# Rajwardhan0511/LLM-Based-Apache-Spark-Optimization

Hardware: AMD Instinct MI355X
Metric: output_tokens_per_sec (higher is better)
Workload: dtype bf16; 1 GPU; model=duckdb-nsql-7B, global_batch=32, seq_len=256, prompt_len=128, parallelism=dp1, decode=greedy

## Files before the change

csrc/bindings.cpp:

```cpp
#ifdef LSA_BINDINGS_SELFTEST
#include <ATen/ATen.h>
#include <hip/hip_runtime_api.h>
#else
#include <torch/extension.h>
#include <c10/hip/HIPStream.h>
#include <hip/hip_runtime.h>
#endif

#include "kernels/gemm_sk.h"
#include "kernels/lsa_epi.h"

extern "C" {
int lsa_gemm(const void* X, int ldx, int M, int K, const void* Wf, int N, void* out, int epi, int nb, int splitk,
             hipStream_t stream);
int lsa_add_rmsnorm(float* h, const float* parts, int nparts, long part_stride, const int* ids, const void* emb,
                    const int* row_idx, int write_h, const void* w, float eps, void* xn, int rows, int D,
                    int xf_mt, long long* ss_out, int ss_ld, int ss_nzero, void* x8, float* sx8, hipStream_t s);
int lsa_prefetch(const void* const* ptrs, const long* bytes, int nr, int wgs, hipStream_t s);
int lsa_res_add_ss(float* h, const float* parts, int nparts, long part_stride, void* xn, int rows, int D, int xf_mt,
                   long long* ss_out, hipStream_t s);
int lsa_a8_gemm(const void* X8, const void* s8, const float* sx, int M, int K, const void* Wq, const float* wscale,
                const void* Sw, int wk, int N, void* out, void* out_s8, int epi, int nb, int splitk, int waves, int depth,
                int xfo, const LsaEpi* ep, hipStream_t stream);
int lsa_quant_xf8(const void* x, int ldx, int M, int K, int MT, void* x8, float* sx, hipStream_t s);
// ... 85 lines not shown
int lsa_ar_alloc(size_t bytes, void** out);
int lsa_ar_free(void* p);
int lsa_ar_handle(void* p, char* out64);
int lsa_ar_open(const char* in64, void** out);
int lsa_ar_close(void* p);
int lsa_ar_max_world();
int lsa_prefill_qblock();
int lsa_ar_wallclock_khz(int* out);
int lsa_ar_header_bytes();
int lsa_ar_run(float* data, long n, float* out, uint8_t* const* regions, int rank, int world, size_t maxb,
               int nblocks, long long timeout_ticks, int* err, int nslab, long slab_stride, const float* res_h,
               void* res_xn, long long* res_ss, int res_d, int res_xmt, int mode, hipStream_t s);
int lsa_fp4_gemm_ex(const void* X, int ldx, int M, int K, const void* Wq, const void* S, int N, void* out, int epi,
                    int nb, int splitk, int waves, int xfrag, const LsaEpi* ep, hipStream_t stream);
int lsa_fp4_dequant(const void* Wq, const void* S, int N, int K, void* Wf, hipStream_t s);
}

namespace {

#ifdef LSA_BINDINGS_SELFTEST
hipStream_t cur_stream() { return nullptr; }
bool on_dev(const at::Tensor& t) { return t.defined(); }
#else
hipStream_t cur_stream() { return c10::hip::getCurrentHIPStream().stream(); }
bool on_dev(const at::Tensor& t) { return t.is_cuda(); }
#endif

void check(int rc, const char* what) { TORCH_CHECK(rc == 0, "lsa kernel '", what, "' failed: rc=", rc); }

void need(const at::Tensor& t, at::ScalarType dt, const char* name) {
// ... 141 lines not shown
             const c10::optional<at::Tensor>& rowss, double eps, const c10::optional<at::Tensor>& h,
             const c10::optional<at::Tensor>& xout, int64_t xmt, const c10::optional<at::Tensor>& ss_out, const c10::optional<at::Tensor>& tickets) {
  need(xf, at::kBFloat16, "xf");
  need(wf, at::kBFloat16, "wf");
  TORCH_CHECK(M >= 1 && M <= 64 && K % 32 == 0, "gemm_xf: M in 1..64, K % 32 == 0");
  const int64_t mt = M <= 16 ? 1 : (M <= 32 ? 2 : 4);
  TORCH_CHECK(xf.is_contiguous() && xf.numel() >= mt * 16 * K, "xf too small for M=", M, " K=", K);
  TORCH_CHECK(wf.numel() == N * K, "weight numel mismatch");
  check_out(epi, out, splitk, M, N, mt);
  const EpiOpts eo = epi_opts(epi, M, N, K, rowss, eps, h, xout, xmt, ss_out, tickets, N / 16);
  check(lsa_gemm_ex(xf.data_ptr(), K, M, K, wf.data_ptr(), N, out.data_ptr(), epi, nb, splitk, waves, div, 2,
                    eo.on ? &eo.e : nullptr, cur_stream()),
        "gemm_xf");
}


void fp8_gemm_xf(const at::Tensor& xf, int64_t M, int64_t K, const at::Tensor& wq, const at::Tensor& wscale, int64_t N,
                 at::Tensor& out, int64_t epi, int64_t nb, int64_t splitk, int64_t waves, int64_t depth,
                 const c10::optional<at::Tensor>& rowss,
                 double eps, const c10::optional<at::Tensor>& h, const c10::optional<at::Tensor>& xout, int64_t xmt,
                 const c10::optional<at::Tensor>& ss_out, const c10::optional<at::Tensor>& tickets) {
  need(xf, at::kBFloat16, "xf");
  need(wscale, at::kFloat, "wscale");
  TORCH_CHECK(on_dev(wq) && wq.element_size() == 1 && wq.numel() == N * K, "wq must be N*K fp8 bytes");
  TORCH_CHECK(M >= 1 && M <= 64 && K % 64 == 0, "fp8_gemm_xf: M in 1..64, K % 64 == 0");
  const int64_t mt = M <= 16 ? 1 : (M <= 32 ? 2 : 4);
  TORCH_CHECK(xf.is_contiguous() && xf.numel() >= mt * 16 * K, "xf too small");
  check_out(epi, out, splitk, M, N, mt);
  const EpiOpts eo = epi_opts(epi, M, N, K, rowss, eps, h, xout, xmt, ss_out, tickets, N / 16);
  lsa_fp8_gemm_knobs((int)waves, (int)depth);
// ... 926 lines not shown
                   (int)res_xmt, (int)mode, cur_stream()),
        "ar_run");
}

}

#ifndef LSA_BINDINGS_SELFTEST
PYBIND11_MODULE(TORCH_EXTENSION_NAME, m) {
  m.doc() = "gfx950 HIP kernels for the MI355X NL->SQL / Spark-error inference engine";
  m.def("gemm", &gemm, py::arg("x"), py::arg("wf"), py::arg("N"), py::arg("out"), py::arg("epi"), py::arg("nb"),
        py::arg("splitk"), py::arg("waves") = 4, py::arg("div") = 4, py::arg("xlds") = 0,
        py::arg("rowss") = py::none(), py::arg("eps") = 1e-5, py::arg("h") = py::none(), py::arg("xout") = py::none(), py::arg("xmt") = 0, py::arg("ss_out") = py::none(), py::arg("tickets") = py::none());
  m.def("gemm_xf", &gemm_xf, py::arg("xf"), py::arg("M"), py::arg("K"), py::arg("wf"), py::arg("N"), py::arg("out"),
        py::arg("epi"), py::arg("nb"), py::arg("splitk"), py::arg("waves") = 4, py::arg("div") = 4,
        py::arg("rowss") = py::none(), py::arg("eps") = 1e-5, py::arg("h") = py::none(), py::arg("xout") = py::none(), py::arg("xmt") = 0, py::arg("ss_out") = py::none(), py::arg("tickets") = py::none());
  m.def("gemm_sk", &gemm_sk, py::arg("x"), py::arg("wf"), py::arg("N"), py::arg("out"), py::arg("epi"), py::arg("ws"),
        py::arg("tickets"), py::arg("ncu"), py::arg("min_share") = 0, py::arg("cfg") = -1, py::arg("xf") = 0,
        py::arg("rows") = 0);
  m.def("gemm_sk_rope", &gemm_sk_rope, py::arg("x"), py::arg("wf"), py::arg("ws"), py::arg("tickets"), py::arg("ncu"),
        py::arg("min_share"), py::arg("cfg"), py::arg("pos"), py::arg("tok_seq"), py::arg("block_tables"),
        py::arg("cos_t"), py::arg("sin_t"), py::arg("q_out"), py::arg("kc"), py::arg("vc"), py::arg("H"), py::arg("Hkv"),
        py::arg("xf") = 0, py::arg("rows") = 0);
  m.def("gemm_sk_epilogue", [](int64_t mode) { lsa_gemm_sk_epilogue((int)mode); });
  m.def("gemm_sk_nbuf", [](int64_t n) { lsa_gemm_sk_nbuf((int)n); });
  m.def("gemm_sk_one_phase", [](int64_t on) { lsa_gemm_sk_one_phase((int)on); });
  m.def("rmsnorm_xf_tile_min", [](int64_t rows) { lsa_rmsnorm_xf_tile_min((int)rows); });
  m.def("gemm_sk_ws_bytes", [](int64_t ncu) { return lsa_gemm_sk_ws_bytes((int)ncu); });
  m.def("gemm_sk_tickets", [](int64_t ncu) { return (int64_t)lsa_gemm_sk_tickets((int)ncu); });
  m.def("fp4_gemm", &fp4_gemm, py::arg("x"), py::arg("wq"), py::arg("sw"), py::arg("N"), py::arg("out"), py::arg("epi"),
        py::arg("nb"), py::arg("splitk"), py::arg("waves") = 4, py::arg("rowss") = py::none(), py::arg("eps") = 1e-5,
// ... 105 lines not shown
```

llm_based_apache_spark_optimization_amd/engine/runner.py:

```python
from __future__ import annotations


import math
import os
from typing import Optional, Sequence

import torch

from .. import ops
from ..models.llama import LlamaWeights
from ..ops import reference as ref

BLOCK = 64
REPEAT_WINDOW = 64
RR_DECODE = os.environ.get("LSA_RR", "1") != "0"


class TPCommError(RuntimeError):
    """A TP peer missed a one-shot all-reduce (the kernel poisoned the result with NaN and set err)."""


class ModelRunner:
    def __init__(self, weights: LlamaWeights, max_slots: int = 32, max_model_len: int = 4096,
                 num_kv_blocks: Optional[int] = None, kv_memory_fraction: float = 0.85,
                 max_new_cap: Optional[int] = None, tp=None, use_graphs: bool = True,
                 fuse_rope: Optional[bool] = None, seq_parallel: Optional[bool] = None, sp_min_tokens: Optional[int] = None,
                 kv_dtype: Optional[str] = None, spec_tokens: int = 0, spec_ngram: tuple = (3, 1),
                 spec_quantized: bool = False, spec_guided: bool = False, spec_sampled: bool = False):
        self.w = weights
        self.spec_tokens = int(spec_tokens)
# ... 102 lines not shown
        a8d = self.a8 and self.a8_down_ok
        self.x8d = torch.zeros(xr * self.ffn_l if a8d else 1, dtype=torch.uint8, device=dev)
        self.s8d = torch.full((mt64 * 64 * (self.ffn_l // 128) if a8d else 1,), 127, dtype=torch.uint8, device=dev)
        self.o_buf = torch.zeros(8 * S * self.d, **f32)
        self.down_buf = torch.zeros(8 * S * self.d, **f32)
        self.qkv_buf = torch.zeros(8 * S * (self.H + 2 * self.Hkv) * self.D, **f32)
        self.logits_l = torch.zeros(S, self.Vl, **f32)
        self.logits = self.logits_l if tps == 1 else torch.zeros(S, self.V, **f32)
        self.gather_buf = None if tps == 1 else torch.zeros(tps * S * self.Vl, **f32)
        nsplit_max = max(4, ops.decode_split_plan(1, self.Hkv, self.max_model_len)[1])
        self.attn_ws = ops.decode_workspace(S, self.H, self.Hkv, nsplit_max, dev)
        self.amax_part = torch.zeros(S * ((self.V + 4095) // 4096), dtype=torch.int64, device=dev)
        self.cand = torch.zeros(S * ((self.V + 2047) // 2048) * 64, dtype=torch.int64, device=dev)
        self.fused_norm = tps == 1 and all(lw.norms_folded for lw in weights.layers)
        self.fused_norm_max_batch = 16 if self.d >= 4096 else 0
        self.res_cfg = None
        self.ssq = torch.zeros(2 * self.L + 2, S, dtype=torch.int64, device=dev)
        self.res_tickets = torch.zeros(max(64, self.d // 16), dtype=torch.int32, device=dev)
        self.wide_norm = all(lw.norms_folded for lw in weights.layers)
        self._plan_rr()
        self.zero_slab = torch.zeros(1, 1, self.d, **f32)
        self.h_alt = torch.zeros(1, self.d, **f32)
        self.graphs: dict = {}
        self._pending_bt: dict = {}
        self.park_past_prompt = False
        self.guided = False
        self._g_host_on: set = set()
        if self.tp is not None and self.tp.size > 1 and self.on_gpu:
            self.tp.warmup()
            if not self.tp.capturable():
# ... 46 lines not shown
    def _a8_splitk_b1(self) -> int:
        kind = self.w.layers[0].wqkv.kind
        if kind not in ("fp8", "mxfp4"):
            return 1
        ak = "fp8a" if kind == "fp8" else "fp4a"
        return max(ops.pick_gemm_config(1, self.d, K, "f32", xf=True, kind=ak)[1] for K in (self.H * self.D, self.ffn_l))

    def oracle_plan(self, B: int) -> dict:
        plan = dict(zip(("qkv", "gate_up", "o", "down"), self.a8_plan(B)))
        plan["rr"] = B == 1 and self.rr_decode and self.rr_a8
        return plan

    def use_xfrag(self, B: int) -> bool:
        return self.on_gpu and 16 < B <= 64 and self.w.layers[0].wqkv.kind in ("bf16", "fp8", "mxfp4")

    def _lm_head(self, xn: torch.Tensor, M: int, xf: bool = False) -> torch.Tensor:
        loc = self.logits_l[:M] if M <= self.max_slots else torch.empty(M, self.Vl, dtype=torch.float32,
                                                                         device=self.device)
        if xf:
            ops.linear_xf(xn, M, self.w.lm_head, "f32", out=loc, splitk=1)
        else:
            ops.linear(xn, self.w.lm_head, "f32", out=loc, splitk=1)
        return self._gather_logits(loc, M)

    def _gather_logits(self, loc: torch.Tensor, M: int) -> torch.Tensor:
        if self.tp is None or self.tp.size == 1:
            return loc
        tps = self.tp.size
        gb = self.gather_buf[: tps * M * self.Vl] if M <= self.max_slots else torch.empty(
            tps * M * self.Vl, dtype=torch.float32, device=self.device)
        self.tp.all_gather(gb, loc.reshape(-1))
        full = self.logits[:M] if M <= self.max_slots else torch.empty(M, self.V, dtype=torch.float32,
                                                                      device=self.device)
        full.view(M, tps, self.Vl).copy_(gb.view(tps, M, self.Vl).transpose(0, 1))
        return full
# ... 29 lines not shown
        wna = self.wide_norm and not a8
        wnm = self.wide_norm and not a8m
        raw0 = wna or wnm
        ssq = self.ssq
        rn_a = lambda l: dict(rownorm=(ssq[2 * l], self.eps)) if (wna or (l == 0 and raw0)) else {}
        assert not (a8 and wna), "a W8A8 qkv input comes from the quantising norm launch"
        rn_m = lambda l: dict(rownorm=(ssq[2 * l + 1], self.eps)) if wnm else {}
        o_parts = self.o_buf[: sk_o * B * d].view(sk_o, B, d)
        d_parts = self.down_buf[: sk_d * B * d].view(sk_d, B, d)
        qkv_parts = self.qkv_buf[: sk_q * B * nqkv].view(sk_q, B, nqkv)
        plan = plan or ops.decode_split_plan(B, self.Hkv, self.max_model_len)
        ws = self.attn_ws
        if xf:
            xn, attn, act = self.xn_f, self.attn_f, self.act_f

            def lin(x, wt, epi, **kw):
                return ops.linear_xf(x, B, wt, epi, **kw)
        else:
            xn, attn, act = self.xn[:B], self.attn[:B], self.act[:B]
            lin = ops.linear
        for l, lw in enumerate(w.layers):
            if l == 0 and raw0:
                ops.add_rmsnorm(h, lw.attn_norm, self.eps, xn, ids=ids, emb=w.embed, rows=B, xf=xf,
                                ss_out=ssq.view(-1), ss_ld=self.max_slots, ss_nzero=2 * self.L, **q8)
            elif l == 0:
                ops.add_rmsnorm(h, lw.attn_norm, self.eps, xn, ids=ids, emb=w.embed, rows=B, xf=xf, **q8)
            elif wna:
                self._reduce_add(d_parts, h, xn, ssq[2 * l], B, xf)
            else:
                ops.add_rmsnorm(h, lw.attn_norm, self.eps, xn, parts=self._reduce_parts(d_parts), rows=B, xf=xf, **q8)
            if a8:
                ops.linear_a8(self.x8, self.sx8, B, lw.wqkv, "f32", out=qkv_parts, splitk=sk_q, **rn_a(l))
            else:
                lin(xn, lw.wqkv, "f32", out=qkv_parts, splitk=sk_q, **rn_a(l))
            kc, vc = self.kv[l, 0], self.kv[l, 1]
# ... 12 lines not shown
                lin(attn, lw.wo, "f32", out=o_parts, splitk=sk_o)
            if wnm:
                self._reduce_add(o_parts, h, xn, ssq[2 * l + 1], B, xf)
            else:
                ops.add_rmsnorm(h, lw.mlp_norm, self.eps, xn, parts=self._reduce_parts(o_parts), rows=B, xf=xf, **q8m)
            if a8m:
                ops.linear_a8(self.x8, self.sx8, B, lw.w_gate_up, "silu", out=self.x8d if a8d else act,
                              out_s8=self.s8d if a8d else None)
            else:
                lin(xn, lw.w_gate_up, "silu", out=act, **rn_m(l))
            if a8d:
                ops.linear_a8(self.x8d, None, B, lw.w_down, "f32", out=d_parts, splitk=sk_d, s8=self.s8d)
            else:
                lin(act, lw.w_down, "f32", out=d_parts, splitk=sk_d)
        ops.add_rmsnorm(h, w.final_norm, self.eps, xn, parts=self._reduce_parts(d_parts), rows=B, xf=xf)
        self._decode_tail(B, sample, xn, xf, guided)

    def _decode_step_fused(self, B: int, sample: bool, plan: Optional[tuple] = None, guided: bool = False) -> None:
        w, d = self.w, self.d
        ids, pos, bt = self.input_ids[:B], self.positions[:B], self.block_tables[:B]
        h = self.h[:B]
        xf = self.use_xfrag(B)
        nqkv = (self.H + 2 * self.Hkv) * self.D
        sk_q = self._splitk(B, d, nqkv, tp_reduced=False, xf=xf)
        sk_o = ops.pick_gemm_config(B, d, self.H * self.D, "res", xf=xf, kind=w.layers[0].wo.kind)[1]
        sk_d = ops.pick_gemm_config(B, d, self.ffn_l, "res", xf=xf, kind=w.layers[0].w_down.kind)[1]
        rc = {}
        if self.res_cfg is not None:
            nb_, sk_o, wv_, dv_ = self.res_cfg
            sk_d = sk_o
            rc = dict(nb=nb_, waves=wv_, div=dv_)
# ... 73 lines not shown
                ops.linear_a8_rr(hs[cur], o_parts, hs[1 - cur], lw.w_gate_up, "silu", out=self.x8d, out_s8=self.s8d,
                                 eps=self.eps)
                cur = 1 - cur
                ops.linear_a8(self.x8d, None, 1, lw.w_down, "f32", out=d_parts, splitk=sk_d, s8=self.s8d)
                continue
            ops.attn_decode(self.q[:1], kc, vc, bt, pos, self.H, self.Hkv, self.scale, attn.view(1, self.H, self.D),
                            workspace=self.attn_ws, plan=plan, qkv_parts=qkv_parts, cos=self.cos, sin=self.sin,
                            kv_scales=self._kv_scales(l), rownorm=rn)
            ops.linear(attn, lw.wo, "f32", out=o_parts, splitk=sk_o)
            ops.linear_rr(hs[cur], o_parts, hs[1 - cur], lw.w_gate_up, "silu", out=act, eps=self.eps)
            cur = 1 - cur
            ops.linear(act, lw.w_down, "f32", out=d_parts, splitk=sk_d)
        ops.add_rmsnorm(hs[cur], w.final_norm, self.eps, xn, parts=d_parts, rows=1, write_h=False)
        self._decode_tail(B, sample, xn, False, guided)

    def _decode_tail(self, B: int, sample: bool, xn, xf: bool, guided: bool = False) -> None:
        logits = self._lm_head(xn, B, xf)
        if guided:
            self._dfa_mask(logits, self.gen_len[:B], self.input_ids[:B], self.finished[:B])
        st = (self.out_tokens[:B], self.gen_len[:B], self.input_ids[:B], self.positions[:B], self.finished[:B])
        if sample:
            ops.sample_commit(logits, self.hist[:B], self.penalty[:B], self.temperature[:B], self.top_k[:B],
                              self.top_p[:B], self.seeds[:B], *st, self.eos, self.limit[:B], self.eos_on[:B],
                              workspace=(self.amax_part, self.cand) if self.on_gpu else None,
                              last_n=self.last_n[:B])
        else:
            ops.argmax_commit(logits, *st, self.eos, self.limit[:B], self.eos_on[:B],
                              part=self.amax_part if self.on_gpu else None)

    def final_hidden(self, B: int) -> torch.Tensor:
        if self.step_xfrag(B):
            return ops.from_xfrag(self.xn_f, B, self.d)
# ... 678 lines not shown
```

llm_based_apache_spark_optimization_amd/models/llama.py:

```python
from __future__ import annotations

import dataclasses
import math
import glob
import json
import os
from typing import Optional

import torch

from .. import ops
from .spec import ModelSpec, spec_from_hf_config


FOLD_NORMS = True


@dataclasses.dataclass
class LayerWeights:
    wqkv: ops.PackedWeight
    wo: ops.PackedWeight
    w_gate_up: ops.PackedWeight
    w_down: ops.PackedWeight
    attn_norm: torch.Tensor
# ... 42 lines not shown
def pack_layer(spec: ModelSpec, wq, wk, wv, wo, wg, wu, wd, an, mn, rank=0, tp=1, kind="bf16") -> LayerWeights:
    hd = spec.head_dim
    hq, hk = spec.n_heads // tp, spec.n_kv_heads // tp
    q = wq.view(spec.n_heads, hd, -1)[rank * hq:(rank + 1) * hq].reshape(hq * hd, -1)
    k = wk.view(spec.n_kv_heads, hd, -1)[rank * hk:(rank + 1) * hk].reshape(hk * hd, -1)
    v = wv.view(spec.n_kv_heads, hd, -1)[rank * hk:(rank + 1) * hk].reshape(hk * hd, -1)
    wqkv = torch.cat([q, k, v], 0)
    wo_s = _shard_cols(wo, rank, tp)
    gu = ops.interleave_gate_up(_shard_rows(wg, rank, tp), _shard_rows(wu, rank, tp))
    wd_s = _shard_cols(wd, rank, tp)
    an, mn = an.to(torch.bfloat16), mn.to(torch.bfloat16)
    if FOLD_NORMS:
        wqkv = (wqkv.float() * an.float()[None, :]).to(torch.bfloat16)
        gu = (gu.float() * mn.float()[None, :]).to(torch.bfloat16)
        an, mn = torch.ones_like(an), torch.ones_like(mn)
    P = ops.PackedWeight.from_dense
    return LayerWeights(P(wqkv.contiguous(), kind), P(wo_s.contiguous(), kind), P(gu.contiguous(), kind),
                        P(wd_s.contiguous(), kind), an.contiguous(),
                        mn.contiguous(), norms_folded=FOLD_NORMS)


def init_random(spec: ModelSpec, device="cpu", seed: int = 0, kind: str = "bf16", std: float = 0.02,
                tp_rank: int = 0, tp_size: int = 1) -> LlamaWeights:
    check_tp(spec, tp_size)
    dev = torch.device(device)
    g = torch.Generator(device=dev).manual_seed(seed)
    d, hd = spec.hidden, spec.head_dim

    def rnd(*shape, s=std):
        return (torch.randn(*shape, generator=g, device=dev, dtype=torch.float32) * s).to(torch.bfloat16)

# ... 3 lines not shown
    embed = rnd(spec.vocab_size, d, s=1.0)
    layers = []
    for _ in range(spec.n_layers):
        wq = rnd(spec.n_heads * hd, d)
        wk = rnd(spec.n_kv_heads * hd, d)
        wv = rnd(spec.n_kv_heads * hd, d)
        wo = rnd(d, spec.n_heads * hd)
        wg = rnd(spec.ffn, d)
        wu = rnd(spec.ffn, d)
        wd = rnd(d, spec.ffn)
        layers.append(pack_layer(spec, wq, wk, wv, wo, wg, wu, wd, ones(d), ones(d), tp_rank, tp_size, kind))
        del wq, wk, wv, wo, wg, wu, wd
    final_norm = ones(d)
    head = embed if spec.tie_embeddings else rnd(spec.vocab_size, d)
    lm_head = ops.PackedWeight.from_dense(_shard_rows(head, tp_rank, tp_size).contiguous(), kind)
    return LlamaWeights(spec, embed, layers, final_norm, lm_head, tp_rank, tp_size)


def from_hf_state_dict(spec: ModelSpec, sd: dict, device="cpu", kind: str = "bf16", tp_rank: int = 0,
                       tp_size: int = 1) -> LlamaWeights:
    check_tp(spec, tp_size)
    dev = torch.device(device)

    def t(name):
        return sd[name].to(device=dev, dtype=torch.bfloat16)

    layers = []
    for i in range(spec.n_layers):
        p = f"model.layers.{i}."
        layers.append(pack_layer(
            spec, t(p + "self_attn.q_proj.weight"), t(p + "self_attn.k_proj.weight"), t(p + "self_attn.v_proj.weight"),
            t(p + "self_attn.o_proj.weight"), t(p + "mlp.gate_proj.weight"), t(p + "mlp.up_proj.weight"),
            t(p + "mlp.down_proj.weight"), t(p + "input_layernorm.weight"), t(p + "post_attention_layernorm.weight"),
            tp_rank, tp_size, kind))
    embed = t("model.embed_tokens.weight").contiguous()
    head = embed if (spec.tie_embeddings or "lm_head.weight" not in sd) else t("lm_head.weight")
    lm_head = ops.PackedWeight.from_dense(_shard_rows(head, tp_rank, tp_size).contiguous(), kind)
    return LlamaWeights(spec, embed, layers, t("model.norm.weight").contiguous(), lm_head, tp_rank, tp_size)


def load_safetensors_dir(path: str, device="cpu", kind="bf16", name: Optional[str] = None,
                         template: Optional[str] = None, tp_rank=0, tp_size=1) -> LlamaWeights:
    from safetensors.torch import load_file

    from .spec import get_spec

    with open(os.path.join(path, "config.json")) as f:
        cfg = json.load(f)
    if template is None:
        try:
            template = get_spec(name).template if name else "raw"
        except KeyError:
# ... 103 lines not shown
```

llm_based_apache_spark_optimization_amd/ops/__init__.py:

```python
from __future__ import annotations

import dataclasses
import importlib
import importlib.util
import json
import math
import os
from typing import NamedTuple, Optional

import torch

from . import reference as ref

_ext = None
_ext_err: Optional[BaseException] = None

EPI = {"bf16": 0, "f32": 1, "silu": 2, "res": 3}


def ext():
    global _ext, _ext_err
    if _ext is None and _ext_err is None:
        try:
            alt = os.environ.get("LSA_HIP_SO")
# ... 124 lines not shown
    sp[:, :kb] = sl
    return wq, sp.view(N // 16, kb4, 4, 64).permute(0, 1, 3, 2).contiguous()


def dequantize_mxfp4(wq: torch.Tensor, sw: torch.Tensor, N: int, K: int) -> torch.Tensor:
    kb = K // 128
    packed = wq.reshape(N // 16, kb, 4, 16, 16).permute(0, 3, 1, 2, 4).reshape(N, K // 2)
    codes = torch.stack([packed & 15, packed >> 4], dim=-1).view(N, K).long()
    vals = torch.tensor(FP4_VALUES, device=wq.device)[codes & 7] * (1.0 - 2.0 * (codes >> 3).float())
    sb = sw.reshape(N // 16, -1, 64, 4).permute(0, 1, 3, 2).reshape(N // 16, -1, 64)[:, :kb]
    sb = sb.reshape(N // 16, kb, 4, 16).permute(0, 3, 1, 2).reshape(N, K // 32).float()
    scale = torch.where(sb > 0, torch.exp2(sb - 127.0), torch.zeros_like(sb))
    return (vals.view(N, K // 32, 32) * scale[..., None]).view(N, K)


@dataclasses.dataclass
class PackedWeight:

    N: int
    K: int
    kind: str
    data: torch.Tensor
    scale: Optional[torch.Tensor] = None
    requested: Optional[str] = None

    @staticmethod
    def from_dense(w: torch.Tensor, kind: str = "bf16") -> "PackedWeight":
        N, K = w.shape
        if not w.is_cuda:
            return PackedWeight(N, K, "dense", w.to(torch.bfloat16).contiguous(), None, kind)
        if kind == "fp8":
            q, s = quantize_fp8(w)
            return PackedWeight(N, K, "fp8", q, s.contiguous())
        if kind == "mxfp4":
            wq, sw = pack_mxfp4(*quantize_mxfp4(w))
            return PackedWeight(N, K, "mxfp4", wq, sw)
        wb = w.to(torch.bfloat16)
        return PackedWeight(N, K, "bf16", shuffle_weight(wb))

# ... 403 lines not shown
def to_xfrag(x: torch.Tensor) -> torch.Tensor:
    M, K = x.shape
    mt = xfrag_tiles(M)
    xp = torch.zeros(mt * 16, K, dtype=x.dtype, device=x.device)
    xp[:M] = x
    return xp.view(mt, 16, K // 32, 4, 8).permute(2, 0, 3, 1, 4).contiguous().view(-1)


def from_xfrag(xf: torch.Tensor, M: int, K: int) -> torch.Tensor:
    mt = xfrag_tiles(M)
    return xf[: mt * 16 * K].view(K // 32, mt, 4, 16, 8).permute(1, 3, 0, 2, 4).reshape(mt * 16, K)[:M]


def linear_xf(xf: torch.Tensor, M: int, w: PackedWeight, epi: str = "bf16", out: Optional[torch.Tensor] = None,
              splitk: Optional[int] = None, nb: Optional[int] = None, waves: Optional[int] = None,
              div: Optional[int] = None, rownorm=None, res=None) -> torch.Tensor:
    if not _gpu(xf) or w.kind not in ("bf16", "fp8", "mxfp4"):
        if epi != "silu":
            return linear(from_xfrag(xf, M, w.K), w, epi, out, splitk, nb, waves, div, rownorm, res, _xf=True)
        y = to_xfrag(linear(from_xfrag(xf, M, w.K), w, epi, None, splitk, nb, waves, div, rownorm))
        if out is None:
            return y
        out.view(-1)[: y.numel()].copy_(y)
        return out
    nb0, sk0, wv0, dv0 = pick_gemm_config(M, w.N, w.K, epi, xf=True, kind=w.kind)
    nb = nb0 if nb is None else nb
    splitk = sk0 if splitk is None else splitk
    waves = wv0 if waves is None else waves
    div = dv0 if div is None else div
    if epi == "res":
        splitk, out = _res_split(res, splitk, out, M, w.N, xf.device)
    if out is None:
        if epi == "f32":
            out = torch.empty(splitk, M, w.N, device=xf.device, dtype=torch.float32)
        elif epi == "silu":
            out = torch.zeros(xfrag_tiles(M) * 16 * (w.N // 2), device=xf.device, dtype=torch.bfloat16)
        else:
            out = torch.empty(M, w.N, device=xf.device, dtype=torch.bfloat16)
    kw = _epi_kw(rownorm, res, xfrag_tiles(M))
    if w.kind == "fp8":
        ext().fp8_gemm_xf(xf, M, w.K, w.data, w.scale, w.N, out, EPI[epi], nb, splitk, waves, _fp8_depth(div), **kw)
    elif w.kind == "mxfp4":
        ext().fp4_gemm_xf(xf, M, w.K, w.data, w.scale, w.N, out, EPI[epi], nb, splitk, waves, **kw)
    else:
        ext().gemm_xf(xf, M, w.K, w.data, w.N, out, EPI[epi], nb, splitk, waves, div, **kw)
    return out


FP8_A8_DECODE = os.environ.get("LSA_FP8_A8", "1") != "0"


def to_xf8(x8: torch.Tensor, mt: int) -> torch.Tensor:
    M, K = x8.shape
    full = torch.zeros(16 * mt, K, dtype=torch.uint8, device=x8.device)
    full[:M] = x8
# ... 648 lines not shown
```

Baseline: 8574 tokens/s.

## Add lossless 12-bit compressed bf16 weight GEMM for batch 17-32 decode

Adds a lossless compression of bf16 weights. Each weight keeps its low mantissa byte, plus a 4-bit code holding the sign and an exponent offset inside an 8-value window. Values whose exponent falls outside the window are stored as escapes and patched in the kernel. A new HIP skinny GEMM decodes these planes on the fly with byte permutes, so decode at batch 17-32 reads about 12 bits per weight instead of 16 and moves less memory in the bandwidth-bound regime. In exchange it adds ALU decode work, escape-patch branches, extra model memory because the dense copy is kept, and a fallback path when blocks have too many escapes.

```diff
diff --git a/csrc/bindings.cpp b/csrc/bindings.cpp
--- a/csrc/bindings.cpp
+++ b/csrc/bindings.cpp
@@ -123,6 +123,8 @@
 int lsa_fp4_gemm_ex(const void* X, int ldx, int M, int K, const void* Wq, const void* S, int N, void* out, int epi,
                     int nb, int splitk, int waves, int xfrag, const LsaEpi* ep, hipStream_t stream);
 int lsa_fp4_dequant(const void* Wq, const void* S, int N, int K, void* Wf, hipStream_t s);
+int lsa_gemm_z12(const void* X, int M, int K, const void* lo, const void* hi, const void* esc, int base, int N,
+                 void* out, int epi, int nb, int splitk, int waves, int div, const LsaEpi* ep, hipStream_t stream);
 }
 
 namespace {
@@ -294,6 +296,30 @@
         "gemm_xf");
 }
 
+void z12_gemm_xf(const at::Tensor& xf, int64_t M, int64_t K, const at::Tensor& lo, const at::Tensor& hi,
+                 const at::Tensor& esc, int64_t base, int64_t N, at::Tensor& out, int64_t epi, int64_t nb,
+                 int64_t splitk, int64_t waves, int64_t div, const c10::optional<at::Tensor>& rowss, double eps) {
+  need(xf, at::kBFloat16, "xf");
+  need(lo, at::kByte, "lo");
+  need(hi, at::kByte, "hi");
+  need(esc, at::kInt, "esc");
+  TORCH_CHECK(M > 16 && M <= 32 && K >= 32 && K % 32 == 0 && N >= 16 && N % 16 == 0,
+              "z12_gemm_xf: M in 17..32, K % 32 == 0, N % 16 == 0");
+  TORCH_CHECK(epi >= 0 && epi <= 2, "z12_gemm_xf: epilogue bf16 (0), f32 (1) or silu (2)");
+  TORCH_CHECK(base >= 1 && base <= 120, "z12_gemm_xf: base out of range");
+  TORCH_CHECK(splitk >= 1 && splitk <= K / 32 && (epi == 1 || splitk == 1), "z12_gemm_xf: bad splitk");
+  TORCH_CHECK(xf.is_contiguous() && xf.numel() >= 2 * 16 * K, "xf too small for M=", M, " K=", K);
+  TORCH_CHECK(lo.is_contiguous() && hi.is_contiguous() && esc.is_contiguous() && lo.numel() == N * K &&
+                  hi.numel() == N * K / 2 && esc.numel() == (N / 16) * (K / 32) * 4,
+              "z12 planes do not match N x K");
+  check_out(epi, out, splitk, M, N, 2);
+  TORCH_CHECK(epi != 2 || out.numel() >= 32 * ((N / 2 + 31) / 32 * 32), "z12_gemm_xf: silu out too small");
+  const EpiOpts eo = epi_opts(epi, M, N, K, rowss, eps, c10::nullopt, c10::nullopt, 0, c10::nullopt, c10::nullopt, 0);
+  check(lsa_gemm_z12(xf.data_ptr(), (int)M, (int)K, lo.data_ptr(), hi.data_ptr(), esc.data_ptr(), (int)base, (int)N,
+                     out.data_ptr(), (int)epi, (int)nb, (int)splitk, (int)waves, (int)div, eo.on ? &eo.e : nullptr,
+                     cur_stream()),
+        "z12_gemm_xf");
+}
 
 void fp8_gemm_xf(const at::Tensor& xf, int64_t M, int64_t K, const at::Tensor& wq, const at::Tensor& wscale, int64_t N,
                  at::Tensor& out, int64_t epi, int64_t nb, int64_t splitk, int64_t waves, int64_t depth,
@@ -1250,6 +1276,9 @@
   m.def("gemm_xf", &gemm_xf, py::arg("xf"), py::arg("M"), py::arg("K"), py::arg("wf"), py::arg("N"), py::arg("out"),
         py::arg("epi"), py::arg("nb"), py::arg("splitk"), py::arg("waves") = 4, py::arg("div") = 4,
         py::arg("rowss") = py::none(), py::arg("eps") = 1e-5, py::arg("h") = py::none(), py::arg("xout") = py::none(), py::arg("xmt") = 0, py::arg("ss_out") = py::none(), py::arg("tickets") = py::none());
+  m.def("z12_gemm_xf", &z12_gemm_xf, py::arg("xf"), py::arg("M"), py::arg("K"), py::arg("lo"), py::arg("hi"),
+        py::arg("esc"), py::arg("base"), py::arg("N"), py::arg("out"), py::arg("epi"), py::arg("nb"), py::arg("splitk"),
+        py::arg("waves") = 4, py::arg("div") = 4, py::arg("rowss") = py::none(), py::arg("eps") = 1e-5);
   m.def("gemm_sk", &gemm_sk, py::arg("x"), py::arg("wf"), py::arg("N"), py::arg("out"), py::arg("epi"), py::arg("ws"),
         py::arg("tickets"), py::arg("ncu"), py::arg("min_share") = 0, py::arg("cfg") = -1, py::arg("xf") = 0,
         py::arg("rows") = 0);
diff --git a/csrc/kernels/gemm_z12.hip b/csrc/kernels/gemm_z12.hip
--- /dev/null
+++ b/csrc/kernels/gemm_z12.hip
@@ -0,0 +1,304 @@
+#include "common.h"
+
+#define EPI_BF16 0
+#define EPI_F32 1
+#define EPI_SILU 2
+
+typedef unsigned int u32x2_t __attribute__((ext_vector_type(2)));
+
+__device__ __forceinline__ uint2 ldg_nt2(const uint2* p) {
+  const u32x2_t v = __builtin_nontemporal_load(reinterpret_cast<const u32x2_t*>(p));
+  return make_uint2(v[0], v[1]);
+}
+__device__ __forceinline__ uint32_t ldg_nt1(const uint32_t* p) { return __builtin_nontemporal_load(p); }
+
+__device__ __forceinline__ uint4 z12_decode(const uint2 lo, const uint32_t hi, const uint32_t base4) {
+  const uint32_t ha = ((hi & 0x07070707u) + base4) | ((hi & 0x08080808u) << 4);
+  const uint32_t hb = (((hi >> 4) & 0x07070707u) + base4) | (hi & 0x80808080u);
+  uint4 r;
+  r.x = __builtin_amdgcn_perm(ha, lo.x, 0x05010400u);
+  r.y = __builtin_amdgcn_perm(ha, lo.x, 0x07030602u);
+  r.z = __builtin_amdgcn_perm(hb, lo.y, 0x05010400u);
+  r.w = __builtin_amdgcn_perm(hb, lo.y, 0x07030602u);
+  return r;
+}
+
+__device__ __forceinline__ void z12_patch1(uint4& w, const uint32_t e, const int lane) {
+  const bool mine = (e >> 31) != 0u && ((e >> 20) & 63u) == (uint32_t)lane;
+  const uint32_t slot = (e >> 16) & 7u, d = slot >> 1;
+  const uint32_t keep = (slot & 1u) ? 0x0000ffffu : 0xffff0000u;
+  const uint32_t ins = (slot & 1u) ? (e << 16) : (e & 0xffffu);
+  w.x = (mine && d == 0u) ? ((w.x & keep) | ins) : w.x;
+  w.y = (mine && d == 1u) ? ((w.y & keep) | ins) : w.y;
+  w.z = (mine && d == 2u) ? ((w.z & keep) | ins) : w.z;
+  w.w = (mine && d == 3u) ? ((w.w & keep) | ins) : w.w;
+}
+
+template <int MT, int NB, int DIV>
+struct Z12Cfg {
+  static constexpr int U0 = (16 / (NB > 2 * MT ? NB : 2 * MT)) < 2 ? 2 : (16 / (NB > 2 * MT ? NB : 2 * MT));
+  static constexpr int U = (U0 / DIV) < 1 ? 1 : (U0 / DIV);
+};
+
+template <int NB, int EPI, int WAVES, int DIV>
+__global__ __launch_bounds__(64 * WAVES) void gemm_z12_kernel(const uint16_t* __restrict__ X, int M, int KB,
+                                                              const uint2* __restrict__ Lo,
+                                                              const uint32_t* __restrict__ Hi,
+                                                              const uint32_t* __restrict__ Esc, uint32_t base4,
+                                                              void* __restrict__ out, int ldo, int kb_per_split,
+                                                              LsaEpi ep) {
+  constexpr int MT = 2;
+  constexpr int U = Z12Cfg<MT, NB, DIV>::U;
+  const int lane = threadIdx.x & 63;
+  const int w = __builtin_amdgcn_readfirstlane(threadIdx.x >> 6);
+  const int r = lane & 15;
+  int nb0, cnt;
+  skinny_nblocks<NB, EPI == EPI_SILU ? 2 : 1>(EPI == EPI_SILU ? ldo / 8 : ldo / 16, nb0, cnt);
+  const int kbA = blockIdx.y * kb_per_split;
+  const int kbB = min(KB, kbA + kb_per_split);
+  const int nk = kbB - kbA;
+  const int nch = (nk + U - 1) / U;
+  const int n_it = nch > w ? (nch - w + WAVES - 1) / WAVES : 0;
+
+  f32x4_t acc[NB][MT];
+#pragma unroll
+  for (int i = 0; i < NB; ++i)
+#pragma unroll
+    for (int j = 0; j < MT; ++j) acc[i][j] = f32x4_t{0.f, 0.f, 0.f, 0.f};
+
+  const uint16_t* xp[MT];
+  bool xvalid[MT];
+#pragma unroll
+  for (int j = 0; j < MT; ++j) {
+    xvalid[j] = j * 16 + r < M;
+    xp[j] = X + ((size_t)j * 64 + lane) * 8;
+  }
+  size_t fb[NB];
+#pragma unroll
+  for (int i = 0; i < NB; ++i) fb[i] = (size_t)(nb0 + min(i, cnt - 1)) * KB;
+
+  struct Chunk {
+    uint2 lo[U][NB];
+    uint32_t hi[U][NB];
+    uint32_t esc[U][NB];
+    uint4 x[U][MT];
+  };
+  auto load = [&](Chunk& c, int ci) {
+    const int kb = kbA + ci * U;
+#pragma unroll
+    for (int u = 0; u < U; ++u) {
+      const int kk = min(kb + u, kbB - 1);
+#pragma unroll
+      for (int i = 0; i < NB; ++i) {
+        const size_t f = fb[i] + kk;
+        c.lo[u][i] = ldg_nt2(Lo + f * 64 + lane);
+        c.hi[u][i] = ldg_nt1(Hi + f * 64 + lane);
+        c.esc[u][i] = Esc[f * 4 + (lane & 3)];
+      }
+    }
+#pragma unroll
+    for (int u = 0; u < U; ++u) {
+      const int kk = min(kb + u, kbB - 1);
+#pragma unroll
+      for (int j = 0; j < MT; ++j) c.x[u][j] = *reinterpret_cast<const uint4*>(xp[j] + (size_t)kk * MT * 512);
+    }
+  };
+  auto comp = [&](const Chunk& c, int ci) {
+    const int kb = kbA + ci * U;
+#pragma unroll
+    for (int u = 0; u < U; ++u) {
+      const bool live = (kb + u) < kbB;
+      uint4 wv[NB];
+#pragma unroll
+      for (int i = 0; i < NB; ++i) {
+        wv[i] = z12_decode(c.lo[u][i], c.hi[u][i], base4);
+        const uint32_t e = c.esc[u][i];
+        if (__builtin_amdgcn_ballot_w64((e >> 31) != 0u)) {
+          z12_patch1(wv[i], __builtin_amdgcn_readlane(e, 0), lane);
+          z12_patch1(wv[i], __builtin_amdgcn_readlane(e, 1), lane);
+          z12_patch1(wv[i], __builtin_amdgcn_readlane(e, 2), lane);
+          z12_patch1(wv[i], __builtin_amdgcn_readlane(e, 3), lane);
+        }
+      }
+#pragma unroll
+      for (int j = 0; j < MT; ++j) {
+        const bool ok = live && xvalid[j];
+        uint4 xv = c.x[u][j];
+        xv.x = ok ? xv.x : 0u; xv.y = ok ? xv.y : 0u; xv.z = ok ? xv.z : 0u; xv.w = ok ? xv.w : 0u;
+#pragma unroll
+        for (int i = 0; i < NB; ++i) acc[i][j] = mfma16x16x32(wv[i], xv, acc[i][j]);
+      }
+    }
+  };
+  auto ch = [&](int i) { return w + WAVES * i; };
+
+  Chunk A, B;
+  if (n_it > 0) {
+    load(A, ch(0));
+    int i = 0;
+    for (; i + 2 < n_it; i += 2) {
+      load(B, ch(i + 1));
+      __builtin_amdgcn_sched_barrier(0);
+      comp(A, ch(i));
+      __builtin_amdgcn_sched_barrier(0);
+      load(A, ch(i + 2));
+      __builtin_amdgcn_sched_barrier(0);
+      comp(B, ch(i + 1));
+      __builtin_amdgcn_sched_barrier(0);
+    }
+    if (i + 1 < n_it) {
+      load(B, ch(i + 1));
+      __builtin_amdgcn_sched_barrier(0);
+      comp(A, ch(i));
+      __builtin_amdgcn_sched_barrier(0);
+      comp(B, ch(i + 1));
+    } else {
+      comp(A, ch(i));
+    }
+  }
+
+  __shared__ __attribute__((aligned(16))) f32x4_t red[WAVES][NB * MT][64];
+#pragma unroll
+  for (int i = 0; i < NB; ++i)
+#pragma unroll
+    for (int j = 0; j < MT; ++j) red[w][i * MT + j][lane] = acc[i][j];
+  __syncthreads();
+
+  if constexpr (EPI == EPI_SILU) {
+    for (int idx = threadIdx.x; idx < (NB / 2) * MT * 64; idx += 64 * WAVES) {
+      const int l = idx & 63;
+      const int t = idx >> 6;
+      const int j = t % MT, p = t / MT;
+      f32x4_t gs = red[0][(2 * p) * MT + j][l], us = red[0][(2 * p + 1) * MT + j][l];
+#pragma unroll
+      for (int ww = 1; ww < WAVES; ++ww) {
+        gs += red[ww][(2 * p) * MT + j][l];
+        us += red[ww][(2 * p + 1) * MT + j][l];
+      }
+      const int m = j * 16 + (l & 15);
+      if (m < M && 2 * p < cnt) {
+        const int n = ((nb0 + 2 * p) >> 1) * 16 + 4 * (l >> 4);
+        const float sc = epi_row_scale(ep, m);
+        f32x4_t v;
+#pragma unroll
+        for (int q = 0; q < 4; ++q) v[q] = silu(gs[q] * sc) * (us[q] * sc);
+        uint2 pk;
+        pk.x = pack2bf(v[0], v[1]);
+        pk.y = pack2bf(v[2], v[3]);
+        *reinterpret_cast<uint2*>(reinterpret_cast<uint16_t*>(out) + xf_off(m, n, MT)) = pk;
+      }
+    }
+  } else {
+    const size_t slab = (size_t)blockIdx.y * M * ldo;
+    for (int idx = threadIdx.x; idx < NB * MT * 64; idx += 64 * WAVES) {
+      const int l = idx & 63;
+      const int t = idx >> 6;
+      const int j = t % MT, i = t / MT;
+      f32x4_t s = red[0][t][l];
+#pragma unroll
+      for (int ww = 1; ww < WAVES; ++ww) s += red[ww][t][l];
+      const int m = j * 16 + (l & 15);
+      if (m < M && i < cnt) {
+        s *= epi_row_scale(ep, m);
+        const int n = (nb0 + i) * 16 + 4 * (l >> 4);
+        if constexpr (EPI == EPI_F32) {
+          float* o = reinterpret_cast<float*>(out) + slab + (size_t)m * ldo + n;
+          *reinterpret_cast<float4*>(o) = make_float4(s[0], s[1], s[2], s[3]);
+        } else {
+          uint2 pk;
+          pk.x = pack2bf(s[0], s[1]);
+          pk.y = pack2bf(s[2], s[3]);
+          *reinterpret_cast<uint2*>(reinterpret_cast<uint16_t*>(out) + (size_t)m * ldo + n) = pk;
+        }
+      }
+    }
+  }
+}
+
+struct Z12Args {
+  const uint16_t* X;
+  int M, KB;
+  const uint2* lo;
+  const uint32_t* hi;
+  const uint32_t* esc;
+  uint32_t base4;
+  int NBtot;
+  void* out;
+  int ldo, splitk, waves, div;
+  LsaEpi ep;
+  hipStream_t s;
+};
+
+template <int NB, int EPI, int WV, int DV>
+static void launch_z12_d(const Z12Args& a) {
+  const int kbps = (a.KB + a.splitk - 1) / a.splitk;
+  dim3 grid((a.NBtot + NB - 1) / NB, a.splitk);
+  hipLaunchKernelGGL((gemm_z12_kernel<NB, EPI, WV, DV>), grid, dim3(64 * WV), 0, a.s, a.X, a.M, a.KB, a.lo, a.hi, a.esc,
+                     a.base4, a.out, a.ldo, kbps, a.ep);
+}
+
+template <int NB, int EPI>
+static void launch_z12_n(const Z12Args& a) {
+  if constexpr (NB >= 6) {
+    if (a.div == 1) launch_z12_d<NB, EPI, 4, 1>(a);
+    else launch_z12_d<NB, EPI, 4, 2>(a);
+  } else if (a.div == 2) {
+    if (a.waves == 8) launch_z12_d<NB, EPI, 8, 2>(a);
+    else launch_z12_d<NB, EPI, 4, 2>(a);
+  } else if (a.div == 4) {
+    launch_z12_d<NB, EPI, 4, 4>(a);
+  } else {
+    if (a.waves == 8) launch_z12_d<NB, EPI, 8, 1>(a);
+    else launch_z12_d<NB, EPI, 4, 1>(a);
+  }
+}
+
+template <int EPI>
+static int launch_z12_e(const Z12Args& a, int nb) {
+  if (nb == 2) launch_z12_n<2, EPI>(a);
+  else if (nb == 4) launch_z12_n<4, EPI>(a);
+  else if (nb == 6) launch_z12_n<6, EPI>(a);
+  else return -2;
+  return 0;
+}
+
+extern "C" int lsa_gemm_z12(const void* X, int M, int K, const void* lo, const void* hi, const void* esc, int base, int N,
+                            void* out, int epi, int nb, int splitk, int waves, int div, const LsaEpi* ep,
+                            hipStream_t stream) {
+  if (K % 32 != 0 || N % 16 != 0 || M <= 16 || M > 32) return -1;
+  if (base < 1 || base > 120) return -1;
+  if (ep && (ep->h || ep->xout || ep->ss_out)) return -8;
+  if (epi != EPI_BF16 && epi != EPI_F32 && epi != EPI_SILU) return -4;
+  const int NBtot = N / 16;
+  if (nb != 2 && nb != 4 && nb != 6) return -2;
+  if (epi == EPI_SILU && NBtot % 2) return -2;
+  if (NBtot % nb != 0 && (epi == EPI_SILU ? NBtot / 2 < (NBtot + nb - 1) / nb : NBtot < (NBtot + nb - 1) / nb))
+    return -2;
+  if (splitk < 1) splitk = 1;
+  if (splitk > K / 32) return -3;
+  if (epi != EPI_F32 && splitk != 1) return -3;
+  Z12Args a;
+  a.X = reinterpret_cast<const uint16_t*>(X);
+  a.M = M;
+  a.KB = K / 32;
+  a.lo = reinterpret_cast<const uint2*>(lo);
+  a.hi = reinterpret_cast<const uint32_t*>(hi);
+  a.esc = reinterpret_cast<const uint32_t*>(esc);
+  a.base4 = (uint32_t)base * 0x01010101u;
+  a.NBtot = NBtot;
+  a.out = out;
+  a.ldo = epi == EPI_SILU ? N / 2 : N;
+  a.splitk = splitk;
+  a.waves = waves == 8 ? 8 : 4;
+  a.div = (div == 1 || div == 2) ? div : 4;
+  a.ep = ep ? *ep : LsaEpi{};
+  a.s = stream;
+  int rc;
+  switch (epi) {
+    case EPI_BF16: rc = launch_z12_e<EPI_BF16>(a, nb); break;
+    case EPI_F32: rc = launch_z12_e<EPI_F32>(a, nb); break;
+    default: rc = launch_z12_e<EPI_SILU>(a, nb); break;
+  }
+  if (rc) return rc;
+  return (int)hipGetLastError();
+}
diff --git a/llm_based_apache_spark_optimization_amd/engine/runner.py b/llm_based_apache_spark_optimization_amd/engine/runner.py
--- a/llm_based_apache_spark_optimization_amd/engine/runner.py
+++ b/llm_based_apache_spark_optimization_amd/engine/runner.py
@@ -14,6 +14,7 @@
 BLOCK = 64
 REPEAT_WINDOW = 64
 RR_DECODE = os.environ.get("LSA_RR", "1") != "0"
+Z12_MAX_BATCH = 32
 
 
 class TPCommError(RuntimeError):
@@ -146,6 +147,7 @@
         self.cand = torch.zeros(S * ((self.V + 2047) // 2048) * 64, dtype=torch.int64, device=dev)
         self.fused_norm = tps == 1 and all(lw.norms_folded for lw in weights.layers)
         self.fused_norm_max_batch = 16 if self.d >= 4096 else 0
+        self.z12_max_batch = Z12_MAX_BATCH
         self.res_cfg = None
         self.ssq = torch.zeros(2 * self.L + 2, S, dtype=torch.int64, device=dev)
         self.res_tickets = torch.zeros(max(64, self.d // 16), dtype=torch.int32, device=dev)
@@ -222,11 +224,11 @@
     def use_xfrag(self, B: int) -> bool:
         return self.on_gpu and 16 < B <= 64 and self.w.layers[0].wqkv.kind in ("bf16", "fp8", "mxfp4")
 
-    def _lm_head(self, xn: torch.Tensor, M: int, xf: bool = False) -> torch.Tensor:
+    def _lm_head(self, xn: torch.Tensor, M: int, xf: bool = False, z12: bool = False) -> torch.Tensor:
         loc = self.logits_l[:M] if M <= self.max_slots else torch.empty(M, self.Vl, dtype=torch.float32,
                                                                          device=self.device)
         if xf:
-            ops.linear_xf(xn, M, self.w.lm_head, "f32", out=loc, splitk=1)
+            ops.linear_xf(xn, M, self.w.lm_head, "f32", out=loc, splitk=1, z12=z12)
         else:
             ops.linear(xn, self.w.lm_head, "f32", out=loc, splitk=1)
         return self._gather_logits(loc, M)
@@ -286,11 +288,14 @@
         if xf:
             xn, attn, act = self.xn_f, self.attn_f, self.act_f
 
+            z12 = 16 < B <= self.z12_max_batch
+
             def lin(x, wt, epi, **kw):
-                return ops.linear_xf(x, B, wt, epi, **kw)
+                return ops.linear_xf(x, B, wt, epi, z12=z12, **kw)
         else:
             xn, attn, act = self.xn[:B], self.attn[:B], self.act[:B]
             lin = ops.linear
+            z12 = False
         for l, lw in enumerate(w.layers):
             if l == 0 and raw0:
                 ops.add_rmsnorm(h, lw.attn_norm, self.eps, xn, ids=ids, emb=w.embed, rows=B, xf=xf,
@@ -333,7 +338,7 @@
             else:
                 lin(act, lw.w_down, "f32", out=d_parts, splitk=sk_d)
         ops.add_rmsnorm(h, w.final_norm, self.eps, xn, parts=self._reduce_parts(d_parts), rows=B, xf=xf)
-        self._decode_tail(B, sample, xn, xf, guided)
+        self._decode_tail(B, sample, xn, xf, guided, z12=z12)
 
     def _decode_step_fused(self, B: int, sample: bool, plan: Optional[tuple] = None, guided: bool = False) -> None:
         w, d = self.w, self.d
@@ -437,8 +442,8 @@
         ops.add_rmsnorm(hs[cur], w.final_norm, self.eps, xn, parts=d_parts, rows=1, write_h=False)
         self._decode_tail(B, sample, xn, False, guided)
 
-    def _decode_tail(self, B: int, sample: bool, xn, xf: bool, guided: bool = False) -> None:
-        logits = self._lm_head(xn, B, xf)
+    def _decode_tail(self, B: int, sample: bool, xn, xf: bool, guided: bool = False, z12: bool = False) -> None:
+        logits = self._lm_head(xn, B, xf, z12)
         if guided:
             self._dfa_mask(logits, self.gen_len[:B], self.input_ids[:B], self.finished[:B])
         st = (self.out_tokens[:B], self.gen_len[:B], self.input_ids[:B], self.positions[:B], self.finished[:B])
diff --git a/llm_based_apache_spark_optimization_amd/models/llama.py b/llm_based_apache_spark_optimization_amd/models/llama.py
--- a/llm_based_apache_spark_optimization_amd/models/llama.py
+++ b/llm_based_apache_spark_optimization_amd/models/llama.py
@@ -80,7 +80,10 @@
         wqkv = (wqkv.float() * an.float()[None, :]).to(torch.bfloat16)
         gu = (gu.float() * mn.float()[None, :]).to(torch.bfloat16)
         an, mn = torch.ones_like(an), torch.ones_like(mn)
-    P = ops.PackedWeight.from_dense
+    def P(w, kind):
+        pw = ops.PackedWeight.from_dense(w, kind)
+        return pw.add_z12() if tp == 1 else pw
+
     return LayerWeights(P(wqkv.contiguous(), kind), P(wo_s.contiguous(), kind), P(gu.contiguous(), kind),
                         P(wd_s.contiguous(), kind), an.contiguous(),
                         mn.contiguous(), norms_folded=FOLD_NORMS)
@@ -114,6 +117,8 @@
     final_norm = ones(d)
     head = embed if spec.tie_embeddings else rnd(spec.vocab_size, d)
     lm_head = ops.PackedWeight.from_dense(_shard_rows(head, tp_rank, tp_size).contiguous(), kind)
+    if tp_size == 1:
+        lm_head.add_z12()
     return LlamaWeights(spec, embed, layers, final_norm, lm_head, tp_rank, tp_size)
 
 
@@ -136,6 +141,8 @@
     embed = t("model.embed_tokens.weight").contiguous()
     head = embed if (spec.tie_embeddings or "lm_head.weight" not in sd) else t("lm_head.weight")
     lm_head = ops.PackedWeight.from_dense(_shard_rows(head, tp_rank, tp_size).contiguous(), kind)
+    if tp_size == 1:
+        lm_head.add_z12()
     return LlamaWeights(spec, embed, layers, t("model.norm.weight").contiguous(), lm_head, tp_rank, tp_size)
 
 
diff --git a/llm_based_apache_spark_optimization_amd/ops/__init__.py b/llm_based_apache_spark_optimization_amd/ops/__init__.py
--- a/llm_based_apache_spark_optimization_amd/ops/__init__.py
+++ b/llm_based_apache_spark_optimization_amd/ops/__init__.py
@@ -162,6 +162,69 @@
     return (vals.view(N, K // 32, 32) * scale[..., None]).view(N, K)
 
 
+Z12 = os.environ.get("LSA_Z12", "1") != "0"
+Z12_WINDOW = 8
+Z12_MAX_ESC = 4
+
+
+class Z12Planes(NamedTuple):
+    lo: torch.Tensor
+    hi: torch.Tensor
+    esc: torch.Tensor
+    base: int
+
+    @property
+    def nbytes(self) -> int:
+        return self.lo.numel() + self.hi.numel() + 4 * self.esc.numel()
+
+
+def z12_base(wf: torch.Tensor) -> int:
+    e7 = (wf.reshape(-1).view(torch.int16).to(torch.int32) >> 8) & 0x7F
+    hist = torch.bincount(e7, minlength=128)[:128].to(torch.int64)
+    c = torch.cat([hist.new_zeros(1), hist.cumsum(0)])
+    cover = c[1 + Z12_WINDOW:129] - c[1:129 - Z12_WINDOW]
+    return int(cover.argmax().item()) + 1
+
+
+def pack_z12(w: torch.Tensor) -> Optional[Z12Planes]:
+    wf = shuffle_weight(w) if w.dim() == 2 else w
+    assert wf.dtype == torch.bfloat16 and wf[0, 0].numel() == 512, (wf.dtype, wf.shape)
+    NB, KB = wf.shape[:2]
+    wf = wf.reshape(NB, KB, 64, 8)
+    base = z12_base(wf)
+    bits = wf.contiguous().view(torch.int16).to(torch.int32) & 0xFFFF
+    hb = bits >> 8
+    e7 = hb & 0x7F
+    out = (e7 < base) | (e7 >= base + Z12_WINDOW)
+    if int(out.sum(dim=(2, 3)).max().item()) > Z12_MAX_ESC:
+        return None
+    code = torch.where(out, torch.zeros_like(hb), ((hb >> 7) << 3) | (e7 - base))
+    lo = (bits & 0xFF).to(torch.uint8)
+    hi = (code[..., :4] | (code[..., 4:] << 4)).to(torch.uint8)
+    esc = torch.zeros(NB * KB, Z12_MAX_ESC, dtype=torch.int64, device=wf.device)
+    idx = out.nonzero()
+    if idx.shape[0]:
+        f = idx[:, 0] * KB + idx[:, 1]
+        first = torch.searchsorted(f, f)
+        rank = torch.arange(f.numel(), device=f.device) - first
+        val = bits[idx[:, 0], idx[:, 1], idx[:, 2], idx[:, 3]].to(torch.int64)
+        esc[f, rank] = (1 << 31) | (idx[:, 2] << 20) | (idx[:, 3] << 16) | val
+    esc = torch.where(esc >= (1 << 31), esc - (1 << 32), esc).to(torch.int32)
+    return Z12Planes(lo.contiguous(), hi.contiguous(), esc.view(NB, KB, Z12_MAX_ESC).contiguous(), base)
+
+
+def unpack_z12(z: Z12Planes) -> torch.Tensor:
+    hi = z.hi.to(torch.int32)
+    code = torch.cat([hi & 0xF, hi >> 4], dim=-1)
+    bits = ((((code & 8) << 4) | ((code & 7) + z.base)) << 8) | z.lo.to(torch.int32)
+    e = z.esc.to(torch.int64) & 0xFFFFFFFF
+    at = (e >> 31).nonzero()
+    if at.shape[0]:
+        ev = e[at[:, 0], at[:, 1], at[:, 2]]
+        bits[at[:, 0], at[:, 1], (ev >> 20) & 63, (ev >> 16) & 7] = (ev & 0xFFFF).to(torch.int32)
+    return torch.where(bits >= 0x8000, bits - 0x10000, bits).to(torch.int16).view(torch.bfloat16)
+
+
 @dataclasses.dataclass
 class PackedWeight:
 
@@ -171,6 +234,12 @@
     data: torch.Tensor
     scale: Optional[torch.Tensor] = None
     requested: Optional[str] = None
+    z12: Optional[Z12Planes] = None
+
+    def add_z12(self) -> "PackedWeight":
+        if Z12 and self.kind == "bf16" and self.z12 is None:
+            self.z12 = pack_z12(self.data)
+        return self
 
     @staticmethod
     def from_dense(w: torch.Tensor, kind: str = "bf16") -> "PackedWeight":
@@ -604,7 +673,7 @@
 
 def linear_xf(xf: torch.Tensor, M: int, w: PackedWeight, epi: str = "bf16", out: Optional[torch.Tensor] = None,
               splitk: Optional[int] = None, nb: Optional[int] = None, waves: Optional[int] = None,
-              div: Optional[int] = None, rownorm=None, res=None) -> torch.Tensor:
+              div: Optional[int] = None, rownorm=None, res=None, z12: bool = False) -> torch.Tensor:
     if not _gpu(xf) or w.kind not in ("bf16", "fp8", "mxfp4"):
         if epi != "silu":
             return linear(from_xfrag(xf, M, w.K), w, epi, out, splitk, nb, waves, div, rownorm, res, _xf=True)
@@ -614,21 +683,32 @@
         out.view(-1)[: y.numel()].copy_(y)
         return out
     nb0, sk0, wv0, dv0 = pick_gemm_config(M, w.N, w.K, epi, xf=True, kind=w.kind)
+    z12 = z12 and w.kind == "bf16" and w.z12 is not None and 16 < M <= 32 and epi in ("bf16", "f32", "silu")
+    if z12:
+        e = _tuning_table().get(f"{w.N}x{w.K}:{epi}:b32:z12")
+        if e is not None and e.get("off"):
+            z12 = nb is not None
+        elif e is not None:
+            nb0, sk0, wv0, dv0 = e["nb"], e["splitk"], e["waves"], e["div"]
     nb = nb0 if nb is None else nb
     splitk = sk0 if splitk is None else splitk
     waves = wv0 if waves is None else waves
     div = dv0 if div is None else div
+    z12 = z12 and nb in (2, 4, 6)
     if epi == "res":
         splitk, out = _res_split(res, splitk, out, M, w.N, xf.device)
     if out is None:
         if epi == "f32":
             out = torch.empty(splitk, M, w.N, device=xf.device, dtype=torch.float32)
         elif epi == "silu":
-            out = torch.zeros(xfrag_tiles(M) * 16 * (w.N // 2), device=xf.device, dtype=torch.bfloat16)
+            out = torch.zeros(xfrag_tiles(M) * 16 * (-(-(w.N // 2) // 32) * 32), device=xf.device, dtype=torch.bfloat16)
         else:
             out = torch.empty(M, w.N, device=xf.device, dtype=torch.bfloat16)
     kw = _epi_kw(rownorm, res, xfrag_tiles(M))
-    if w.kind == "fp8":
+    if z12:
+        z = w.z12
+        ext().z12_gemm_xf(xf, M, w.K, z.lo, z.hi, z.esc, z.base, w.N, out, EPI[epi], nb, splitk, waves, div, **kw)
+    elif w.kind == "fp8":
         ext().fp8_gemm_xf(xf, M, w.K, w.data, w.scale, w.N, out, EPI[epi], nb, splitk, waves, _fp8_depth(div), **kw)
     elif w.kind == "mxfp4":
         ext().fp4_gemm_xf(xf, M, w.K, w.data, w.scale, w.N, out, EPI[epi], nb, splitk, waves, **kw)
```

Result: faster. 8865 tokens/s (median of 6 runs) (+3.4%).
